# daac-tools/daachorse

Hardware: NVIDIA H100
Metric: input GB/s scanned, find_overlapping_iter, 675k-pat bytewise (higher is better)
Workload: dtype u8

## Files before the change

daachorse_b200/csrc/dev_image.cpp:

```cpp
#include "dev_image.h"

#include <algorithm>

namespace dach {

namespace {

bool fail_chains_terminate(const dach_pma* p, bool dead_is_terminal) {
    const size_t n = p->slots();
    std::vector<uint8_t> color(n, 0);
    std::vector<uint32_t> path;
    for (size_t start = 0; start < n; ++start) {
        if (color[start]) continue;
        path.clear();
        uint32_t s = uint32_t(start);
        for (;;) {
            if (s == kRoot || (dead_is_terminal && s == kDead) || color[s] == 2) break;
            if (color[s] == 1) return false;
            color[s] = 1;
            path.push_back(s);
            s = p->fail[s];
        }
        for (uint32_t v : path) color[v] = 2;
    }
// ... 155 lines not shown
        if (s != kRoot && s != kDead && !moved[s]) R->new_of_old[s] = uint32_t(s) + H;
        if (!rebased[s] && p->base[s] != 0) R->new_base[s] = p->base[s] + H;
    }
    R->vacant_check.assign(H, 0);
    for (uint32_t blk = 0; blk < H; blk += 256) {
        uint32_t ub = blk == 0 ? 0u : kNone;
        for (uint32_t b = blk; ub == kNone && b < blk + 256; ++b)
            if (!base_used[b]) {
                ub = b;
                break;
            }
        for (uint32_t v = blk; v < blk + 256; ++v)
            if (!used[v] || v == kRoot || v == kDead) R->vacant_check[v] = ub == kNone ? 0x100u : (0x100u | ((ub ^ v) & 0xffu));
    }
    R->hot_slots = H;
}

}

int build_image(const dach_pma* p, HostImage* img) {
    const size_t n = p->slots();
    const bool lm = is_leftmost(p->match_kind);
    img->charwise = p->charwise;
    img->match_kind = p->match_kind;
    img->n_slots = uint32_t(n);
    img->root_opos = n ? p->state_output_pos(kRoot) : 0;
    img->max_pattern_len = 0;
    for (const OutputRec& o : p->outputs)
        if (o.length > img->max_pattern_len) img->max_pattern_len = o.length;

// ... 76 lines not shown
                uint32_t check = p->opos_ch[s] & 0xffu;
                if (ns < H && R.vacant_check[ns]) check = R.vacant_check[ns] & 0xffu;
                r[0] = (R.new_base[s] << 8) | check;
                r[1] = (nid(f) << 8) | flags;
                const uint32_t list = opos ? img->outputs[(size_t)(opos - 1) * 4 + 3] : 0u;
                r[2] = (fbase << 8) | std::min<uint32_t>(list, 255u);
                r[3] = R.sig[s];
                img->opos_tab[ns] = opos;
            }
            for (uint32_t v = 0; v < H; ++v)
                if (R.vacant_check[v] && v != kRoot && v != kDead) img->crec[size_t(v) * 4] = R.vacant_check[v] & 0xffu;
            if (H)
                for (size_t s = 0; s < n; ++s)
                    if (R.new_of_old[s] < H) img->crec[(s + H) * 4] = p->opos_ch[s] & 0xffu;
        }
    } else {
        for (size_t s = 0; s < n; ++s) {
            uint32_t* r = &img->rec[s * 4];
            r[0] = p->base[s];
            r[1] = p->check[s];
            r[2] = p->fail[s];
            r[3] = p->output_pos[s];
        }
        img->root_table.assign(256, kRoot);
        img->mapper = p->mapper_table;
        img->root_base = n ? p->base[kRoot] : 0;
        if (n < (size_t(1) << 24) && p->outputs.size() < (size_t(1) << 24)) {
            auto skip_leaves = [&](uint32_t f) {
                while (f != kRoot && f != kDead && p->base[f] == 0) f = p->fail[f];
                return f;
// ... 34 lines not shown
```

daachorse_b200/csrc/dev_image.h:

```cpp
#pragma once

#include <cstdint>
#include <vector>

#include "host.h"

namespace dach {

struct HostImage {
    bool charwise = false;
    uint8_t match_kind = 0;
    uint32_t n_slots = 0;
    uint32_t root_opos = 0;
    uint32_t max_pattern_len = 0;
    std::vector<uint32_t> rec;
    std::vector<uint32_t> outputs;
    std::vector<uint32_t> root_table;
    std::vector<uint32_t> crec;
    std::vector<uint32_t> opos_tab;
    uint32_t root_base = 0;
    uint32_t want_hot_slots = 65536;
    uint32_t hot_slots = 0;
    uint32_t n_cslots = 0;
    std::vector<uint32_t> new_of_old;
    std::vector<uint32_t> old_of_new;
    std::vector<uint32_t> mapper;
    bool segmentable = false;
};

int build_image(const dach_pma* p, HostImage* img);

}
```

daachorse_b200/csrc/dev_scan.cu:

```cuda
#include <cuda_runtime.h>

#include <unistd.h>

#include <algorithm>
#include <atomic>
#include <chrono>
#include <cstdio>
#include <cstdlib>
#include <cstring>
#include <memory>
#include <mutex>
#include <string>
#include <vector>

#include "dev_image.h"
#include "host.h"
#include "scan_lane.cuh"

namespace dach {


constexpr int kMaxThreads = 1024;
constexpr int kMaxDevices = 64;
constexpr uint32_t kRootBytes = 1024;
// ... 167 lines not shown
                    }
                }
            }
        }
    }
    if constexpr (SINK::KIND == RK_HIST) {
        __syncthreads();
        for (uint32_t i = threadIdx.x; i < P.hist_smem; i += blockDim.x)
            if (E.s_cnt[i]) red_add_u64(P.slot_hist + i, E.s_cnt[i]);
    }
}

template <class M, class LANE, int MAXT, int MINB, bool HOT>
__global__ void __launch_bounds__(MAXT, MINB) k_scan_machine(ScanParams P) {
    if constexpr (M::QLEN)
        scan_machine<M, EventOps<M::ITER>, LANE, EventSink, HOT>(P);
    else
        scan_machine<M, M, LANE, Emitter, HOT>(P);
}
template <class M, class LANE, int MODE, int RK, bool HOT>
__global__ void __launch_bounds__(1024, 1) k_scan_machine_rk(ScanParams P) {
    scan_machine<M, SinkOps<M, MODE, RK>, LANE, SinkOf<RK>, HOT>(P);
}

template <int MODE, int MAXT, bool HOT>
__global__ void __launch_bounds__(MAXT, 1) k_scan_duo(ScanParams P) {
    using M = StdMachine3<MODE>;
    extern __shared__ __align__(128) unsigned char smem_raw[];
    uint4* s_hot = reinterpret_cast<uint4*>(smem_raw);
    QEntry* s_queue = reinterpret_cast<QEntry*>(smem_raw + (HOT ? (size_t)P.hot_entries * 16 : 0));
    __shared__ __align__(8) uint64_t s_bar;
// ... 598 lines not shown
    DevBuf counts, ev_counts, tiles, ctrl, pool;
    DevBuf nseg, seg_first, item_hay, item_beg, item_offs, n_items_dev;
    DevBuf blk_first, blkmap, tiles2;
    DevBuf stage;
    DevBuf items_rk, total_rk;
    DevBuf slot_hist, rec_hist, hist_acc;
    HostPinned* pinned = nullptr;
    cudaEvent_t ev[4] = {nullptr, nullptr, nullptr, nullptr};
    cudaEvent_t ev_scanned = nullptr, ev_placed = nullptr;
    cudaEvent_t ev_push[2] = {nullptr, nullptr};
    uint64_t job_n = 0, job_items = 0;
    uint32_t job_pool_blocks = 0;
    uint64_t job_cap = 0;
    bool job_seg = false, job_ordered = false, job_open = false, job_placed = false;
    bool job_events = false;
    bool refused = false;
    int job_mode = 0;
    cudaStream_t job_stream = nullptr;
    DevBuf text, offs, out, out_offs;
    void* offs_stage = nullptr;
    size_t offs_stage_bytes = 0;
    cudaStream_t stream = nullptr;
    bool init(bool with_stream) {
        if (!pinned && !cuda_ok(cudaMallocHost(reinterpret_cast<void**>(&pinned), sizeof(HostPinned)), "cudaMallocHost"))
            return false;
        for (int i = 0; i < 4; ++i)
            if (!ev[i] && !cuda_ok(cudaEventCreate(&ev[i]), "cudaEventCreate")) return false;
        if (!ev_scanned && !cuda_ok(cudaEventCreateWithFlags(&ev_scanned, cudaEventDisableTiming), "cudaEventCreate")) return false;
        if (!ev_placed && !cuda_ok(cudaEventCreateWithFlags(&ev_placed, cudaEventDisableTiming), "cudaEventCreate")) return false;
        for (int i = 0; i < 2; ++i)
// ... 44 lines not shown
    bool segmentable = false;
    uint32_t n_outputs = 0, max_value = 0, n_cslots = 0;
    size_t image_bytes = 0;
    int sm_count = 0;
    size_t smem_optin = 0;
    uint4* d_rec = nullptr;
    uint4* d_outputs = nullptr;
    uint32_t* d_root = nullptr;
    uint4* d_crec = nullptr;
    uint32_t* d_opos = nullptr;
    uint32_t* d_id_in = nullptr;
    uint32_t* d_id_out = nullptr;
    uint32_t hot_slots = 0;
    uint32_t root_base = 0;
    uint32_t* d_mapper = nullptr;
    void* image_base = nullptr;
    size_t image_alloc = 0;
    std::mutex mu;
    Workspace ws;
    static constexpr int kSlots = 4;
    Workspace slot[kSlots];
    int64_t opt_slice_mib = 64;
    int64_t opt_hot_entries = 6144;
    int64_t opt_hist_smem = 1024;
    int64_t opt_df_pairs = kDefaultDfPairs;
    int64_t opt_slice_ramp = 1;
    int64_t opt_tail_seg = 0;
    int64_t opt_gather_ordered = 1;
    int64_t opt_gather_u = 4;
    int64_t opt_reserve_sms = 0;
    int64_t opt_smem_pad_kib = 0;
    int64_t opt_seg_len = 0;
    int64_t opt_hot_records = 0;
    int64_t opt_threads = 1024;
    int64_t opt_ctas_per_sm = 1;
    int64_t opt_l2_hints = 2;
    int64_t opt_kernel = 3;
    std::atomic<uint64_t> launches{0};
    cudaEvent_t ev_ref = nullptr;
    double last_scan_ms = 0, last_total_ms = 0;
    uint64_t last_h2d = 0, last_d2h = 0;
    DevBuf df_tab[2], df_list[2], df_n, df_acc;
    uint32_t df_mask = 0, df_limit = 0;
    bool df_clean = false;
    uint64_t last_df_windows = 0, last_df_rescans = 0;
    std::atomic<int> refs{1};
};

struct dach_job {
    dach_dev* d = nullptr;
    Workspace W;
// ... 83 lines not shown
    return cudaGetLastError();
}
template <int MAXT, bool HOT>
cudaError_t launch_duo_m(int mode, const ScanParams& P, int grid, int threads, size_t smem, cudaStream_t st) {
    switch (mode) {
        case M_FIND: return launch_duo_t<M_FIND, MAXT, HOT>(P, grid, threads, smem, st);
        case M_NO_SUFFIX: return launch_duo_t<M_NO_SUFFIX, MAXT, HOT>(P, grid, threads, smem, st);
        case M_OVERLAPPING: return launch_duo_t<M_OVERLAPPING, MAXT, HOT>(P, grid, threads, smem, st);
    }
    return cudaErrorInvalidValue;
}
cudaError_t launch_duo(int mode, const ScanParams& P, int grid, int threads, size_t smem, cudaStream_t st) {
    if (threads > 768)
        return P.hot_entries ? launch_duo_m<1024, true>(mode, P, grid, threads, smem, st) : launch_duo_m<1024, false>(mode, P, grid, threads, smem, st);
    return P.hot_entries ? launch_duo_m<768, true>(mode, P, grid, threads, smem, st) : launch_duo_m<768, false>(mode, P, grid, threads, smem, st);
}

cudaError_t launch_cw(int mode, const ScanParams& P, int grid, int threads, size_t smem, cudaStream_t st) {
    switch (mode) {
        case M_FIND: return launch_machine_t<CwMachine<M_FIND>, LaneCw, 1024, 1, false>(P, grid, threads, smem, st);
        case M_OVERLAPPING: return launch_machine_t<CwMachine<M_OVERLAPPING>, LaneCw, 1024, 1, false>(P, grid, threads, smem, st);
        case M_NO_SUFFIX: return launch_machine_t<CwMachine<M_NO_SUFFIX>, LaneCw, 1024, 1, false>(P, grid, threads, smem, st);
        default: return launch_machine_t<CwMachine<M_LEFTMOST>, LaneCw, 1024, 1, false>(P, grid, threads, smem, st);
    }
}

cudaError_t launch_lm(const ScanParams& P, int grid, int threads, size_t smem, cudaStream_t st) {
    return launch_machine_t<LmMachine, LaneLm, 1024, 1, false>(P, grid, threads, smem, st);
}

// ... 121 lines not shown
    P.mapper = d->d_mapper;
    P.mapper_len = d->mapper_len;
    P.n_slots = d->n_slots;
    P.id_in = d->d_id_in;
    P.id_out = d->d_id_out;
    P.root_opos = d->root_opos;
    P.text = d_text;
    P.text_lo = text_lo;
    P.text_end = text_end;
    P.offs = d_offs;
    P.n_items = n;
    return P;
}

size_t plan_smem(const dach_dev* d, ScanParams& P, bool v1, bool std3, int threads, int ctas_per_sm, int queue_sets,
                 uint32_t hist_smem = 0) {
    const size_t smem_budget = std::min<size_t>(d->smem_optin, 226 * 1024) / ctas_per_sm - (ctas_per_sm > 1 ? 1024 : 0);
    size_t smem;
    if (v1) {
        const size_t queues = (size_t)LANE_Q * threads * sizeof(QEntry) * queue_sets + (size_t)hist_smem * 4;
        uint64_t want = 0;
        if (std3 && d->opt_hot_entries != 0 && smem_budget > queues + 512) {
            want = std::min<uint64_t>(d->hot_slots, (smem_budget - queues - 512) / 16);
            if (d->opt_hot_entries > 0) want = std::min<uint64_t>(want, (uint64_t)d->opt_hot_entries);
            want &= ~uint64_t(255);
        }
        smem = (size_t)want * 16 + queues;
        if (d->opt_smem_pad_kib > 0) smem = std::min<size_t>(smem + ((size_t)d->opt_smem_pad_kib << 10), smem_budget);
        P.hot_n = 0;
        P.hot_entries = (uint32_t)want;
    } else {
        uint64_t hot = smem_budget > kRootBytes ? (smem_budget - kRootBytes) / 16 : 0;
        if (d->opt_hot_records >= 0) hot = std::min<uint64_t>(hot, (uint64_t)d->opt_hot_records);
        hot = std::min<uint64_t>(hot, d->n_slots);
        P.hot_n = (uint32_t)hot;
        smem = kRootBytes + (size_t)hot * 16;
    }
    return smem;
// ... 48 lines not shown
        cudaEventRecord(W.ev_scanned, st);
        return DACH_OK;
    }
    int threads = (int)std::min<int64_t>(std::max<int64_t>(d->opt_threads, 32), kMaxThreads);
    threads = (threads / 32) * 32;
    int ctas_per_sm = (int)std::min<int64_t>(std::max<int64_t>(d->opt_ctas_per_sm, 1), 2048 / threads);
    const int free_sms = (int)std::min<int64_t>(std::max<int64_t>(d->opt_reserve_sms, 0), d->sm_count - 1);
    const int grid = (d->sm_count - free_sms) * ctas_per_sm;
    const bool v1 = d->opt_kernel >= 1 && d->d_crec && !(mode == M_FIND && d->root_opos != 0);
    const bool cw_machine = v1 && d->charwise;
    const bool lm_machine = v1 && !d->charwise && mode == M_LEFTMOST;
    const bool std2 = v1 && !d->charwise && mode != M_LEFTMOST && d->opt_kernel >= 2 && d->root_base != 0;
    const bool std3 = std2 && d->opt_kernel >= 3;
    const bool duo = std3 && d->opt_kernel >= 4 && ctas_per_sm == 1;
    const bool events = std3 && !duo;

    if (d_state_io && !std2 && !cw_machine) {
        set_error("stream chunks need a Standard lane machine (find / find_overlapping, at most 2^24 states, bytewise: "
                  "BASE(ROOT) != 0, no empty pattern for find)");
        return DACH_INVALID_ARGUMENT;
    }

    bool seg = v1 && !d->charwise && !d_state_io && (mode == M_OVERLAPPING || mode == M_NO_SUFFIX) && d->opt_seg_len >= 0 && d->segmentable;
    uint32_t seg_len = 0, seg_from = 0;
    uint64_t n_items_max = n;
    if (seg) {
        const uint64_t lanes = (uint64_t)grid * threads;
        const uint64_t warm = d->max_pattern_len ? d->max_pattern_len - 1 : 0;
        const uint64_t floor_len = std::max<uint64_t>(256, 8 * warm);
        uint64_t want;
// ... 26 lines not shown
    const uint32_t pool_blocks = (uint32_t)pool_blocks64;
    if (!ensure(W.counts, n_items_max * 4) || !ensure(W.tiles, n_tiles * 8) || !ensure(W.item_offs, (n_items_max + 1) * 8) ||
        !ensure(W.pool, (size_t)pool_blocks * BLK_WORDS * 4) || (events && !ensure(W.ev_counts, n_items_max * 4)))
        return DACH_CUDA_ERROR;
    if (seg && (!ensure(W.nseg, n * 4) || !ensure(W.seg_first, (n + 1) * 8) || !ensure(W.item_hay, n_items_max * 4) ||
                !ensure(W.item_beg, n_items_max * 4) || !ensure(W.n_items_dev, 8)))
        return DACH_CUDA_ERROR;

    ScanParams P = image_params(d, d_text, text_lo, text_end, d_offs, n);
    P.counts = static_cast<uint32_t*>(W.counts.p);
    P.ev_counts = events ? static_cast<uint32_t*>(W.ev_counts.p) : nullptr;
    P.pool = static_cast<uint32_t*>(W.pool.p);
    P.pool_blocks = pool_blocks;
    P.ctrl = static_cast<ScanCtrl*>(W.ctrl.p);
    P.state_io = d_state_io;
    const size_t smem = plan_smem(d, P, v1, std3, threads, ctas_per_sm, duo ? 2 : 1);

    unsigned long long* tiles = static_cast<unsigned long long*>(W.tiles.p);
    unsigned long long* item_offs = static_cast<unsigned long long*>(W.item_offs.p);
    k_check_offsets<<<(unsigned)((n + 255) / 256), 256, 0, st>>>(d_offs, n, (uint64_t)(text_end - d_text), P.ctrl);
    ++d->launches;
    if (seg) {
        cudaMemsetAsync(W.counts.p, 0, n_items_max * 4, st);
        if (events) cudaMemsetAsync(W.ev_counts.p, 0, n_items_max * 4, st);
        enqueue_seg_table(d, W, d_offs, n, seg_len, seg_from, P, st);
    }
    cudaEventRecord(W.ev[3], st);
    if (!cuda_ok(cw_machine   ? launch_cw(mode, P, grid, std::min(threads, 1024), smem, st)
                 : lm_machine ? launch_lm(P, grid, std::min(threads, 1024), smem, st)
                 : duo        ? launch_duo(mode, P, grid, threads, smem, st)
                 : v1         ? launch_std(std3 ? 3 : std2 ? 2 : 1, mode, P, grid, threads, smem, st,
                                           ctas_per_sm >= 2 && threads <= 768 && grid % 2 == 0)
                              : launch_scan(d->charwise, mode, P, grid, threads, smem, st),
                 "k_scan launch"))
        return DACH_CUDA_ERROR;
    cudaEventRecord(W.ev[1], st);
    k_offsets_tile_sums<1><<<(unsigned)n_tiles, kScanThreads, 0, st>>>(P.counts, n_items_max, tiles);
    k_offsets_scan_tiles<<<1, kScanThreads, 0, st>>>(tiles, n_tiles);
    k_offsets_apply<1><<<(unsigned)n_tiles, kScanThreads, 0, st>>>(P.counts, n_items_max, tiles, item_offs);
    d->launches += 4;
    const bool ordered = d->opt_gather_ordered >= 2 || (d->opt_gather_ordered == 1 && text_bytes >= (256ull << 20));
    if (ordered) {
        if (!ensure(W.blk_first, (n_items_max + 1) * 8) || !ensure(W.blkmap, (size_t)pool_blocks * 4) || !ensure(W.tiles2, n_tiles * 8))
// ... 6 lines not shown
            k_offsets_apply<BLK_EVENTS><<<(unsigned)n_tiles, kScanThreads, 0, st>>>(P.ev_counts, n_items_max, tiles2, blk_first);
        } else {
            k_offsets_tile_sums<BLK_MATCHES><<<(unsigned)n_tiles, kScanThreads, 0, st>>>(P.counts, n_items_max, tiles2);
            k_offsets_scan_tiles<<<1, kScanThreads, 0, st>>>(tiles2, n_tiles);
            k_offsets_apply<BLK_MATCHES><<<(unsigned)n_tiles, kScanThreads, 0, st>>>(P.counts, n_items_max, tiles2, blk_first);
        }
        k_blk_index<<<d->sm_count * 8, 256, 0, st>>>(P.pool, P.ctrl, pool_blocks, blk_first, static_cast<uint32_t*>(W.blkmap.p));
        d->launches += 4;
    }
    if (!cuda_ok(cudaGetLastError(), "kernel launch")) return DACH_CUDA_ERROR;
    cudaEventRecord(W.ev_scanned, st);
    W.job_items = n_items_max;
    W.job_seg = seg;
    W.job_ordered = ordered;
    W.job_events = events;
    W.job_mode = mode;
    W.job_pool_blocks = pool_blocks;
    return DACH_OK;
}

int enqueue_place(dach_dev* d, Workspace& W, dach_match* d_out, uint64_t out_cap, uint64_t* d_out_offs,
                  const unsigned long long* d_base, bool last, cudaStream_t st, const uint32_t* d_pos_in = nullptr,
                  bool staged = false, bool dma = false, uint64_t h_base = 0, uint64_t h_total = 0) {
    if (!W.job_open) {
        set_error("no scan to place");
        return DACH_INVALID_ARGUMENT;
    }
    if (st != W.job_stream) cudaStreamWaitEvent(st, W.ev_scanned, 0);
    const uint64_t n = W.job_n, n_items = W.job_items;
    const ScanCtrl* ctrl = static_cast<const ScanCtrl*>(W.ctrl.p);
// ... 4 lines not shown
        const uint32_t* pool = static_cast<const uint32_t*>(W.pool.p);
        const uint32_t* counts = static_cast<const uint32_t*>(W.counts.p);
        const uint32_t* blkmap = W.job_ordered ? static_cast<const uint32_t*>(W.blkmap.p) : nullptr;
        uint32_t* out_words = reinterpret_cast<uint32_t*>(d_out);
        const unsigned long long* g_base = d_base;
        unsigned long long g_cap = out_cap;
        if (staged) {
            if (!ensure(W.stage, W.job_cap * sizeof(dach_match) + 256)) return DACH_CUDA_ERROR;
            out_words = static_cast<uint32_t*>(W.stage.p);
            g_base = nullptr;
            g_cap = W.job_cap;
        }
        const unsigned long long* pad_like = staged ? d_base : nullptr;
        if (W.job_events) {
            const uint32_t* ev_counts = static_cast<const uint32_t*>(W.ev_counts.p);
            if (W.job_mode == M_OVERLAPPING)
                k_expand<true, 2><<<gather_grid, 256, 0, st>>>(pool, ctrl, W.job_pool_blocks, ev_counts, item_offs, n_items, g_cap, g_base,
                                                                out_words, blkmap, pad_like, d->d_outputs, d->d_opos);
            else
                k_expand<false, 2><<<gather_grid, 256, 0, st>>>(pool, ctrl, W.job_pool_blocks, ev_counts, item_offs, n_items, g_cap, g_base,
                                                                 out_words, blkmap, pad_like, d->d_outputs, d->d_opos);
        } else if (d->opt_gather_u >= 8)
            k_gather<8><<<gather_grid, 256, 0, st>>>(pool, ctrl, W.job_pool_blocks, counts, item_offs, n_items, g_cap, g_base, out_words, blkmap, pad_like);
        else if (d->opt_gather_u <= 2)
            k_gather<2><<<gather_grid, 256, 0, st>>>(pool, ctrl, W.job_pool_blocks, counts, item_offs, n_items, g_cap, g_base, out_words, blkmap, pad_like);
        else
            k_gather<4><<<gather_grid, 256, 0, st>>>(pool, ctrl, W.job_pool_blocks, counts, item_offs, n_items, g_cap, g_base, out_words, blkmap, pad_like);
        ++d->launches;
        if (staged) {
            cudaEventRecord(W.ev_push[0], st);
            if (dma) {
                if (h_total && h_base + h_total <= out_cap &&
                    !cuda_ok(cudaMemcpyAsync(reinterpret_cast<uint32_t*>(d_out) + h_base * 3ull, out_words + ((h_base * 3ull) & 3ull),
                                             h_total * sizeof(dach_match), cudaMemcpyDefault, st),
                             "peer copy"))
                    return DACH_CUDA_ERROR;
// ... 734 lines not shown
        d->device = device;
        d->charwise = img.charwise;
        d->match_kind = img.match_kind;
        d->n_slots = img.n_slots;
        d->root_opos = img.root_opos;
        d->max_pattern_len = img.max_pattern_len;
        d->segmentable = img.segmentable;
        d->mapper_len = (uint32_t)img.mapper.size();
        d->n_outputs = (uint32_t)(img.outputs.size() / 4);
        for (uint32_t i = 0; i < d->n_outputs; ++i) d->max_value = std::max(d->max_value, img.outputs[(size_t)i * 4]);
        d->n_cslots = (uint32_t)img.opos_tab.size();
        cudaDeviceProp prop;
        if (!cuda_ok(cudaGetDeviceProperties(&prop, device), "cudaGetDeviceProperties")) return DACH_CUDA_ERROR;
        d->sm_count = prop.multiProcessorCount;
        d->smem_optin = prop.sharedMemPerBlockOptin;
        constexpr int kParts = 8;
        const std::vector<uint32_t>* parts[kParts] = {&img.rec, &img.outputs, &img.root_table, &img.mapper, &img.crec, &img.opos_tab,
                                                       &img.new_of_old, &img.old_of_new};
        size_t part_off[kParts], total = 0;
        for (int i = 0; i < kParts; ++i) {
            part_off[i] = total;
            total += (std::max<size_t>(parts[i]->size() * 4, 16) + 511) & ~size_t(511);
            d->image_bytes += parts[i]->size() * 4;
        }
        bool ok = cuda_ok(cudaMalloc(&d->image_base, total), "cudaMalloc image");
        d->image_alloc = total;
        for (int i = 0; ok && i < kParts; ++i)
            if (!parts[i]->empty())
                ok = cuda_ok(cudaMemcpy(static_cast<char*>(d->image_base) + part_off[i], parts[i]->data(), parts[i]->size() * 4,
                                        cudaMemcpyHostToDevice),
                             "upload image");
        if (ok) {
            char* b = static_cast<char*>(d->image_base);
            d->d_rec = reinterpret_cast<uint4*>(b + part_off[0]);
            d->d_outputs = reinterpret_cast<uint4*>(b + part_off[1]);
            d->d_root = reinterpret_cast<uint32_t*>(b + part_off[2]);
            d->d_mapper = reinterpret_cast<uint32_t*>(b + part_off[3]);
            if (!img.crec.empty()) {
                d->d_crec = reinterpret_cast<uint4*>(b + part_off[4]);
                d->d_opos = reinterpret_cast<uint32_t*>(b + part_off[5]);
                if (img.hot_slots) {
                    d->d_id_in = reinterpret_cast<uint32_t*>(b + part_off[6]);
                    d->d_id_out = reinterpret_cast<uint32_t*>(b + part_off[7]);
                }
                d->hot_slots = img.hot_slots;
            }
            d->root_base = img.root_base;
        }
        ok = ok && install_policies((int)d->opt_l2_hints) && d->ws.init(false);
        if (!ok) {
            dach_dev_free(d.release());
            return DACH_CUDA_ERROR;
        }
        *out = d.release();
        return DACH_OK;
    });
}

void dach_dev_free(dach_dev* d) {
    if (!d || --d->refs > 0) return;
    DeviceGuard g(d->device);
    cudaFree(d->image_base);
// ... 523 lines not shown
        d->opt_tail_seg = value;
    else if (k == "gather_ordered")
        d->opt_gather_ordered = value;
    else if (k == "gather_u")
        d->opt_gather_u = value;
    else if (k == "reserve_sms")
        d->opt_reserve_sms = value;
    else if (k == "smem_pad_kib")
        d->opt_smem_pad_kib = value;
    else if (k == "hot_entries")
        d->opt_hot_entries = value;
    else if (k == "hist_smem")
        d->opt_hist_smem = value;
    else if (k == "df_pairs")
        d->opt_df_pairs = value;
    else if (k == "l2_hints") {
        d->opt_l2_hints = value;
        DeviceGuard g(d->device);
        if (!g.ok || !install_policies((int)value)) return DACH_CUDA_ERROR;
    } else {
        set_error("unknown option " + k);
        return DACH_INVALID_ARGUMENT;
    }
    return DACH_OK;
}

}
```

daachorse_b200/csrc/scan_lane.cuh:

```cuda
#pragma once

#include <stdint.h>

#include <type_traits>

#if defined(__CUDACC__)
#define DACH_HD __host__ __device__ __forceinline__
#else
#define DACH_HD inline
#ifndef DACH_EMU_TYPES
#define DACH_EMU_TYPES
struct uint4 {
    uint32_t x, y, z, w;
};
struct uint2 {
    uint32_t x, y;
};
#endif
#endif

#if defined(__CUDA_ARCH__)
#define DACH_SYNCWARP() __syncwarp()
#else
#define DACH_SYNCWARP()
// ... 1913 lines not shown
                L.sig = x.w;
                L.addr = st;
            }
            return;
        }
        if (MODE != M_FIND && (Ev.root_flags & CF_OUT) && beg == 0) {
            QEntry e;
            e.end = 0;
            e.opos = MODE == M_OVERLAPPING ? D_ROOT | (Ev.root_rec.z << 24) : D_ROOT;
            Ev.q[0] = e;
            L.qn = 1;
        }
    }
};

template <class M, int MODE, int RK>
struct SinkOps {
    using Sink = typename std::conditional<
        RK == RK_COUNT, CountSink,
        typename std::conditional<RK == RK_FIRST, FirstSink, typename std::conditional<RK == RK_HIST, HistSink, DfSink>::type>::type>::type;

    template <class LANE>
    static DACH_HD void begin_item(LANE& L, const ScanParams& P, const StdEnv& Ev, Sink& E, uint64_t item, const uint8_t* emu_lo) {
        Emitter unused;
        M::begin_item(L, P, Ev, unused, item, emu_lo);
        E.begin((uint32_t)item);
        if constexpr (RK == RK_DF) {
            if (P.item_hay) E.hay = P.item_hay[item];
        }
        if constexpr (RK == RK_FIRST) {
// ... 30 lines not shown
            L.qn = 0;
        } else {
            if (L.qn == (uint32_t)LANE_Q) {
                const QEntry e = Ev.q[(LANE_Q - 1) * Ev.q_stride];
                if (e.end >= L.from) {
                    emit_head(P, E, ld_u32(Ev.opos + (e.opos & QSLOT_MASK)), e.end);
                    L.fl |= F_DONE | M::IDLE;
                }
            }
            if (!(L.fl & F_DONE)) L.qn = (uint32_t)LANE_Q - 1;
        }
        if (!(L.fl & F_DONE)) L.fl &= ~M::IDLE;
    }
};

template <int MODE>
struct EventOps {
    using M = StdMachine3<MODE>;

    static DACH_HD void begin_item(Lane3& L, const ScanParams& P, const StdEnv& Ev, EventSink& E, uint64_t item,
                                   const uint8_t* emu_lo) {
        Emitter unused;
        M::begin_item(L, P, Ev, unused, item, emu_lo);
        E.begin((uint32_t)item);
    }

    static DACH_HD uint32_t reportable(const Lane3& L, const StdEnv& Ev) {
        uint32_t n = 0;
        for (uint32_t j = 0; j < (uint32_t)LANE_Q; ++j)
            if (j < L.qn && Ev.q[j * Ev.q_stride].end >= L.from) ++n;
        return n;
    }
    static DACH_HD bool need_block(const Lane3& L, const StdEnv& Ev, const EventSink& E) {
        return reportable(L, Ev) > BLK_EVENTS - E.fill;
    }

    static DACH_HD void drain(Lane3& L, const StdEnv& Ev, const ScanParams& P, EventSink& E, uint32_t blk) {
        for (uint32_t j = 0; j < (uint32_t)LANE_Q; ++j) {
            if (j < L.qn) {
                const QEntry e = Ev.q[j * Ev.q_stride];
                if (e.end >= L.from) {
                    if (E.fill == BLK_EVENTS) E.open(P, blk);
                    if (E.blk) st_stream_u2(E.blk + BLK_HDR_WORDS + 2 * E.fill, e.end, e.opos);
                    ++E.fill;
                    ++E.nev;
                    const uint32_t c = E.count + (MODE == M_OVERLAPPING ? qentry_len(P, Ev.opos, e.opos) : 1u);
                    if (c < E.count) count_carry(P);
                    E.count = c;
                }
            }
        }
        L.qn = 0;
// ... 6 lines not shown
```

Measured before the change: 122.9.

## Add UTF-8 codepoint-level automaton and lane machine for bytewise scans

Builds a second double-array automaton at the host whose transitions consume whole UTF-8 codepoints, remapped to frequency-ordered codes, when the bytewise trie is valid UTF-8 and the byte/boundary state ratio is high enough. A new Utf8Machine lane decodes one codepoint per step from a sliding 32-byte register window and walks this compressed trie, so fewer dependent state fetches are needed per input byte, and the smaller table fits the shared-memory hot cache better. It costs extra decode ALU work per step and a more complex host build, and it only applies to non-leftmost event-mode scans when the heuristic or option allows it.

```diff
diff --git a/daachorse_b200/csrc/dev_image.cpp b/daachorse_b200/csrc/dev_image.cpp
--- a/daachorse_b200/csrc/dev_image.cpp
+++ b/daachorse_b200/csrc/dev_image.cpp
@@ -193,6 +193,208 @@
             if (!used[v] || v == kRoot || v == kDead) R->vacant_check[v] = ub == kNone ? 0x100u : (0x100u | ((ub ^ v) & 0xffu));
     }
     R->hot_slots = H;
+}
+
+void build_utf8_image(const dach_pma* p, HostImage* img) {
+    const size_t n = p->slots();
+    img->u8_ok = false;
+    if (is_leftmost(p->match_kind) || n < 2 || img->root_opos != 0 || !img->segmentable) return;
+    auto child = [&](uint32_t s, uint32_t c) -> uint32_t {
+        const uint32_t b = p->base[s], ci = b ^ c;
+        return (b != 0 && ci < n && (p->opos_ch[ci] & 0xffu) == c) ? ci : kNone;
+    };
+    std::vector<uint8_t> rem(n, 0xff), lo(n, 0x80), hi(n, 0xbf);
+    std::vector<uint32_t> acc(n, 0), begin(n, kNone), bfs;
+    std::vector<uint32_t> cpar(n, kNone), cpt(n, 0);
+    bfs.push_back(kRoot);
+    rem[kRoot] = 0;
+    for (size_t h = 0; h < bfs.size(); ++h) {
+        const uint32_t s = bfs[h];
+        if (p->base[s] == 0) continue;
+        const uint32_t from = rem[s] == 0 ? s : begin[s];
+        for (uint32_t c = 0; c < 256; ++c) {
+            const uint32_t ci = child(s, c);
+            if (ci == kNone) continue;
+            uint32_t r;
+            if (rem[s] == 0) {
+                if (c < 0x80) {
+                    r = 0, acc[ci] = c;
+                } else if (c >= 0xc2 && c <= 0xdf) {
+                    r = 1, acc[ci] = c & 0x1f;
+                } else if (c >= 0xe0 && c <= 0xef) {
+                    r = 2, acc[ci] = c & 0x0f, lo[ci] = c == 0xe0 ? 0xa0 : 0x80, hi[ci] = c == 0xed ? 0x9f : 0xbf;
+                } else if (c >= 0xf0 && c <= 0xf4) {
+                    r = 3, acc[ci] = c & 0x07, lo[ci] = c == 0xf0 ? 0x90 : 0x80, hi[ci] = c == 0xf4 ? 0x8f : 0xbf;
+                } else {
+                    return;
+                }
+            } else {
+                if (c < lo[s] || c > hi[s]) return;
+                r = rem[s] - 1u;
+                acc[ci] = (acc[s] << 6) | (c & 0x3f);
+            }
+            rem[ci] = (uint8_t)r;
+            if (r == 0) {
+                cpar[ci] = from;
+                cpt[ci] = acc[ci];
+                begin[ci] = ci;
+            } else {
+                begin[ci] = from;
+            }
+            bfs.push_back(ci);
+        }
+    }
+    std::vector<uint32_t> bnd;
+    for (uint32_t s : bfs) {
+        if (rem[s] != 0) {
+            if (p->opos_ch[s] >> 8) return;
+            continue;
+        }
+        const uint32_t f = p->fail[s];
+        if (s != kRoot && (f >= n || rem[f] != 0)) return;
+        bnd.push_back(s);
+    }
+    if (bnd.size() < 2) return;
+    img->u8_ratio = double(bfs.size()) / double(bnd.size());
+
+    std::vector<std::pair<uint32_t, uint32_t>> freq;
+    {
+        std::vector<uint32_t> cps;
+        for (size_t i = 1; i < bnd.size(); ++i) cps.push_back(cpt[bnd[i]]);
+        std::sort(cps.begin(), cps.end());
+        for (size_t i = 0; i < cps.size();) {
+            size_t j = i;
+            while (j < cps.size() && cps[j] == cps[i]) ++j;
+            freq.push_back({uint32_t(j - i), cps[i]});
+            i = j;
+        }
+        std::stable_sort(freq.begin(), freq.end(), [](const std::pair<uint32_t, uint32_t>& a, const std::pair<uint32_t, uint32_t>& b) {
+            return a.first > b.first;
+        });
+    }
+    const uint32_t n_codes = uint32_t(freq.size());
+    if (n_codes >= 0xffffu) return;
+    uint32_t max_cp = 0;
+    for (auto& f : freq) max_cp = std::max(max_cp, f.second);
+    std::vector<uint32_t> mapper(size_t(max_cp) + 2, n_codes);
+    for (uint32_t k = 0; k < n_codes; ++k) mapper[freq[k].second] = k;
+
+    std::vector<uint32_t> code(n, 0), nch(n, 0), depth(n, 0), sub(n, 0);
+    for (size_t i = 1; i < bnd.size(); ++i) {
+        const uint32_t s = bnd[i];
+        code[s] = mapper[cpt[s]];
+        ++nch[cpar[s]];
+        depth[s] = depth[cpar[s]] + 1;
+    }
+    for (size_t i = bnd.size(); i-- > 0;) {
+        const uint32_t s = bnd[i];
+        sub[s] += 1;
+        if (s != kRoot) sub[cpar[s]] += sub[s];
+    }
+    std::vector<uint32_t> kid_off(n + 1, 0), kids(bnd.size() - 1);
+    for (size_t s = 0; s < n; ++s) kid_off[s + 1] = kid_off[s] + nch[s];
+    {
+        std::vector<uint32_t> fill(kid_off.begin(), kid_off.end() - 1);
+        for (size_t i = 1; i < bnd.size(); ++i) kids[fill[cpar[bnd[i]]]++] = bnd[i];
+    }
+    std::vector<uint32_t> par;
+    for (uint32_t s : bnd)
+        if (nch[s]) {
+            std::sort(kids.begin() + kid_off[s], kids.begin() + kid_off[s + 1], [&](uint32_t a, uint32_t b) { return code[a] < code[b]; });
+            par.push_back(s);
+        }
+    std::stable_sort(par.begin(), par.end(), [&](uint32_t a, uint32_t b) {
+        if (depth[a] != depth[b]) return depth[a] < depth[b];
+        return uint64_t(sub[a]) * nch[b] > uint64_t(sub[b]) * nch[a];
+    });
+
+    std::vector<uint32_t> nxt, nbase(n, 0), nid(n, kNone);
+    auto grow = [&](size_t want) {
+        size_t old = nxt.size();
+        if (want <= old) return;
+        want = std::max(want, old * 2);
+        nxt.resize(want);
+        for (size_t v = old; v < want; ++v) nxt[v] = uint32_t(v);
+    };
+    auto find = [&](uint32_t v) {
+        grow(size_t(v) + 2);
+        while (nxt[v] != v) {
+            nxt[v] = nxt[nxt[v]];
+            v = nxt[v];
+        }
+        return v;
+    };
+    auto is_free = [&](uint32_t v) { return find(v) == v; };
+    grow(size_t(n_codes) + 1024);
+    nxt[0] = 1;
+    nid[kRoot] = 0;
+    uint32_t top = 0, max_base = 0;
+    for (uint32_t s : par) {
+        const uint32_t* ks = &kids[kid_off[s]];
+        const uint32_t m = nch[s], kmin = code[ks[0]];
+        uint32_t b = kNone, v = find(kmin), tries = 0;
+        for (;;) {
+            const uint32_t cand = v - kmin;
+            bool ok = true;
+            for (uint32_t j = 1; ok && j < m; ++j) ok = is_free(cand + code[ks[j]]);
+            if (ok) {
+                b = cand;
+                break;
+            }
+            if (++tries > (1u << 20)) {
+                b = top + 1 - kmin;
+                break;
+            }
+            v = find(v + 1);
+        }
+        grow(size_t(b) + n_codes + 2);
+        nbase[s] = b;
+        max_base = std::max(max_base, b);
+        for (uint32_t j = 0; j < m; ++j) {
+            const uint32_t slot = b + code[ks[j]];
+            nxt[slot] = slot + 1;
+            nid[ks[j]] = slot;
+            top = std::max(top, slot);
+        }
+    }
+    const size_t N = std::max<size_t>(size_t(top) + 1, size_t(max_base) + n_codes + 1);
+    if (N >= kU24Max) return;
+
+    auto skip_leaves = [&](uint32_t f) {
+        while (f != kRoot && nch[f] == 0) f = p->fail[f];
+        return f;
+    };
+    img->u8_root_base = nbase[kRoot];
+    img->u8_codes = n_codes;
+    img->u8_crec.assign(N * 4, 0);
+    img->u8_opos.assign(N, 0);
+    img->u8_of_old.assign(n, kNone);
+    for (size_t v = 0; v < N; ++v) img->u8_crec[v * 4 + 3] = 0xffffffu << 8;
+    for (uint32_t s : bnd) {
+        const uint32_t ns = nid[s];
+        const uint32_t opos = p->opos_ch[s] >> 8;
+        const uint32_t f = skip_leaves(p->fail[s]);
+        uint32_t flags = opos ? 1u : 0u, fbase;
+        if (s == kRoot || f == kRoot) {
+            flags |= 8u;
+            fbase = img->u8_root_base;
+        } else {
+            fbase = nbase[f];
+            if (skip_leaves(p->fail[f]) == kRoot) flags |= 2u;
+        }
+        uint32_t sig = 0;
+        for (uint32_t j = kid_off[s]; j < kid_off[s + 1]; ++j) sig |= 1u << (code[kids[j]] & 15u);
+        const uint32_t list = opos ? img->outputs[(size_t)(opos - 1) * 4 + 3] : 0u;
+        uint32_t* r = &img->u8_crec[size_t(ns) * 4];
+        r[0] = (nbase[s] << 8) | (sig & 0xffu);
+        r[1] = (nid[f] << 8) | flags;
+        r[2] = (fbase << 8) | std::min<uint32_t>(list, 255u);
+        r[3] = ((s == kRoot ? 0xffffffu : nid[cpar[s]]) << 8) | (sig >> 8);
+        img->u8_opos[ns] = opos;
+        img->u8_of_old[s] = ns;
+    }
+    img->u8_mapper.swap(mapper);
+    img->u8_ok = true;
 }
 
 }
@@ -299,6 +501,7 @@
                 for (size_t s = 0; s < n; ++s)
                     if (R.new_of_old[s] < H) img->crec[(s + H) * 4] = p->opos_ch[s] & 0xffu;
         }
+        build_utf8_image(p, img);
     } else {
         for (size_t s = 0; s < n; ++s) {
             uint32_t* r = &img->rec[s * 4];
diff --git a/daachorse_b200/csrc/dev_image.h b/daachorse_b200/csrc/dev_image.h
--- a/daachorse_b200/csrc/dev_image.h
+++ b/daachorse_b200/csrc/dev_image.h
@@ -26,6 +26,14 @@
     std::vector<uint32_t> old_of_new;
     std::vector<uint32_t> mapper;
     bool segmentable = false;
+    bool u8_ok = false;
+    double u8_ratio = 0;
+    uint32_t u8_root_base = 0;
+    uint32_t u8_codes = 0;
+    std::vector<uint32_t> u8_crec;
+    std::vector<uint32_t> u8_opos;
+    std::vector<uint32_t> u8_mapper;
+    std::vector<uint32_t> u8_of_old;
 };
 
 int build_image(const dach_pma* p, HostImage* img);
diff --git a/daachorse_b200/csrc/dev_scan.cu b/daachorse_b200/csrc/dev_scan.cu
--- a/daachorse_b200/csrc/dev_scan.cu
+++ b/daachorse_b200/csrc/dev_scan.cu
@@ -205,7 +205,7 @@
 template <class M, class LANE, int MAXT, int MINB, bool HOT>
 __global__ void __launch_bounds__(MAXT, MINB) k_scan_machine(ScanParams P) {
     if constexpr (M::QLEN)
-        scan_machine<M, EventOps<M::ITER>, LANE, EventSink, HOT>(P);
+        scan_machine<M, EventOps<M::ITER, M, LANE>, LANE, EventSink, HOT>(P);
     else
         scan_machine<M, M, LANE, Emitter, HOT>(P);
 }
@@ -834,6 +834,7 @@
     uint64_t job_cap = 0;
     bool job_seg = false, job_ordered = false, job_open = false, job_placed = false;
     bool job_events = false;
+    bool job_u8 = false;
     bool refused = false;
     int job_mode = 0;
     cudaStream_t job_stream = nullptr;
@@ -908,6 +909,11 @@
     uint32_t hot_slots = 0;
     uint32_t root_base = 0;
     uint32_t* d_mapper = nullptr;
+    uint4* d_u8_crec = nullptr;
+    uint32_t* d_u8_opos = nullptr;
+    uint32_t* d_u8_mapper = nullptr;
+    uint32_t u8_slots = 0, u8_mapper_len = 0, u8_root_base = 0;
+    double u8_ratio = 0;
     void* image_base = nullptr;
     size_t image_alloc = 0;
     std::mutex mu;
@@ -929,6 +935,7 @@
     int64_t opt_threads = 1024;
     int64_t opt_ctas_per_sm = 1;
     int64_t opt_l2_hints = 2;
+    int64_t opt_utf8_stride = -1;
     int64_t opt_kernel = 3;
     std::atomic<uint64_t> launches{0};
     cudaEvent_t ev_ref = nullptr;
@@ -1042,6 +1049,21 @@
     if (threads > 768)
         return P.hot_entries ? launch_duo_m<1024, true>(mode, P, grid, threads, smem, st) : launch_duo_m<1024, false>(mode, P, grid, threads, smem, st);
     return P.hot_entries ? launch_duo_m<768, true>(mode, P, grid, threads, smem, st) : launch_duo_m<768, false>(mode, P, grid, threads, smem, st);
+}
+
+cudaError_t launch_utf8(int mode, const ScanParams& P, int grid, int threads, size_t smem, cudaStream_t st) {
+    switch (mode) {
+        case M_FIND:
+            return P.hot_entries ? launch_machine_t<Utf8Machine<M_FIND>, Lane8, 1024, 1, true>(P, grid, threads, smem, st)
+                                 : launch_machine_t<Utf8Machine<M_FIND>, Lane8, 1024, 1, false>(P, grid, threads, smem, st);
+        case M_NO_SUFFIX:
+            return P.hot_entries ? launch_machine_t<Utf8Machine<M_NO_SUFFIX>, Lane8, 1024, 1, true>(P, grid, threads, smem, st)
+                                 : launch_machine_t<Utf8Machine<M_NO_SUFFIX>, Lane8, 1024, 1, false>(P, grid, threads, smem, st);
+        case M_OVERLAPPING:
+            return P.hot_entries ? launch_machine_t<Utf8Machine<M_OVERLAPPING>, Lane8, 1024, 1, true>(P, grid, threads, smem, st)
+                                 : launch_machine_t<Utf8Machine<M_OVERLAPPING>, Lane8, 1024, 1, false>(P, grid, threads, smem, st);
+    }
+    return cudaErrorInvalidValue;
 }
 
 cudaError_t launch_cw(int mode, const ScanParams& P, int grid, int threads, size_t smem, cudaStream_t st) {
@@ -1193,14 +1215,14 @@
 }
 
 size_t plan_smem(const dach_dev* d, ScanParams& P, bool v1, bool std3, int threads, int ctas_per_sm, int queue_sets,
-                 uint32_t hist_smem = 0) {
+                 uint32_t hist_smem = 0, bool u8 = false) {
     const size_t smem_budget = std::min<size_t>(d->smem_optin, 226 * 1024) / ctas_per_sm - (ctas_per_sm > 1 ? 1024 : 0);
     size_t smem;
     if (v1) {
         const size_t queues = (size_t)LANE_Q * threads * sizeof(QEntry) * queue_sets + (size_t)hist_smem * 4;
         uint64_t want = 0;
         if (std3 && d->opt_hot_entries != 0 && smem_budget > queues + 512) {
-            want = std::min<uint64_t>(d->hot_slots, (smem_budget - queues - 512) / 16);
+            want = std::min<uint64_t>(u8 ? d->u8_slots : d->hot_slots, (smem_budget - queues - 512) / 16);
             if (d->opt_hot_entries > 0) want = std::min<uint64_t>(want, (uint64_t)d->opt_hot_entries);
             want &= ~uint64_t(255);
         }
@@ -1279,6 +1301,8 @@
     const bool std3 = std2 && d->opt_kernel >= 3;
     const bool duo = std3 && d->opt_kernel >= 4 && ctas_per_sm == 1;
     const bool events = std3 && !duo;
+    const bool u8 = events && !d_state_io && d->d_u8_crec &&
+                    (d->opt_utf8_stride > 0 || (d->opt_utf8_stride < 0 && d->u8_ratio >= 1.5));
 
     if (d_state_io && !std2 && !cw_machine) {
         set_error("stream chunks need a Standard lane machine (find / find_overlapping, at most 2^24 states, bytewise: "
@@ -1335,7 +1359,14 @@
     P.pool_blocks = pool_blocks;
     P.ctrl = static_cast<ScanCtrl*>(W.ctrl.p);
     P.state_io = d_state_io;
-    const size_t smem = plan_smem(d, P, v1, std3, threads, ctas_per_sm, duo ? 2 : 1);
+    if (u8) {
+        P.crec = d->d_u8_crec;
+        P.opos_tab = d->d_u8_opos;
+        P.root_base = d->u8_root_base;
+        P.mapper = d->d_u8_mapper;
+        P.mapper_len = d->u8_mapper_len;
+    }
+    const size_t smem = plan_smem(d, P, v1, std3, threads, ctas_per_sm, duo ? 2 : 1, 0, u8);
 
     unsigned long long* tiles = static_cast<unsigned long long*>(W.tiles.p);
     unsigned long long* item_offs = static_cast<unsigned long long*>(W.item_offs.p);
@@ -1347,7 +1378,8 @@
         enqueue_seg_table(d, W, d_offs, n, seg_len, seg_from, P, st);
     }
     cudaEventRecord(W.ev[3], st);
-    if (!cuda_ok(cw_machine   ? launch_cw(mode, P, grid, std::min(threads, 1024), smem, st)
+    if (!cuda_ok(u8           ? launch_utf8(mode, P, grid, threads, smem, st)
+                 : cw_machine ? launch_cw(mode, P, grid, std::min(threads, 1024), smem, st)
                  : lm_machine ? launch_lm(P, grid, std::min(threads, 1024), smem, st)
                  : duo        ? launch_duo(mode, P, grid, threads, smem, st)
                  : v1         ? launch_std(std3 ? 3 : std2 ? 2 : 1, mode, P, grid, threads, smem, st,
@@ -1384,6 +1416,7 @@
     W.job_seg = seg;
     W.job_ordered = ordered;
     W.job_events = events;
+    W.job_u8 = u8;
     W.job_mode = mode;
     W.job_pool_blocks = pool_blocks;
     return DACH_OK;
@@ -1418,12 +1451,13 @@
         const unsigned long long* pad_like = staged ? d_base : nullptr;
         if (W.job_events) {
             const uint32_t* ev_counts = static_cast<const uint32_t*>(W.ev_counts.p);
+            const uint32_t* opos = W.job_u8 ? d->d_u8_opos : d->d_opos;
             if (W.job_mode == M_OVERLAPPING)
                 k_expand<true, 2><<<gather_grid, 256, 0, st>>>(pool, ctrl, W.job_pool_blocks, ev_counts, item_offs, n_items, g_cap, g_base,
-                                                                out_words, blkmap, pad_like, d->d_outputs, d->d_opos);
+                                                                out_words, blkmap, pad_like, d->d_outputs, opos);
             else
                 k_expand<false, 2><<<gather_grid, 256, 0, st>>>(pool, ctrl, W.job_pool_blocks, ev_counts, item_offs, n_items, g_cap, g_base,
-                                                                 out_words, blkmap, pad_like, d->d_outputs, d->d_opos);
+                                                                 out_words, blkmap, pad_like, d->d_outputs, opos);
         } else if (d->opt_gather_u >= 8)
             k_gather<8><<<gather_grid, 256, 0, st>>>(pool, ctrl, W.job_pool_blocks, counts, item_offs, n_items, g_cap, g_base, out_words, blkmap, pad_like);
         else if (d->opt_gather_u <= 2)
@@ -2188,9 +2222,10 @@
         if (!cuda_ok(cudaGetDeviceProperties(&prop, device), "cudaGetDeviceProperties")) return DACH_CUDA_ERROR;
         d->sm_count = prop.multiProcessorCount;
         d->smem_optin = prop.sharedMemPerBlockOptin;
-        constexpr int kParts = 8;
-        const std::vector<uint32_t>* parts[kParts] = {&img.rec, &img.outputs, &img.root_table, &img.mapper, &img.crec, &img.opos_tab,
-                                                       &img.new_of_old, &img.old_of_new};
+        constexpr int kParts = 11;
+        const std::vector<uint32_t>* parts[kParts] = {&img.rec,        &img.outputs,    &img.root_table, &img.mapper,
+                                                       &img.crec,       &img.opos_tab,   &img.new_of_old, &img.old_of_new,
+                                                       &img.u8_crec,    &img.u8_opos,    &img.u8_mapper};
         size_t part_off[kParts], total = 0;
         for (int i = 0; i < kParts; ++i) {
             part_off[i] = total;
@@ -2220,6 +2255,15 @@
                 d->hot_slots = img.hot_slots;
             }
             d->root_base = img.root_base;
+            if (img.u8_ok) {
+                d->d_u8_crec = reinterpret_cast<uint4*>(b + part_off[8]);
+                d->d_u8_opos = reinterpret_cast<uint32_t*>(b + part_off[9]);
+                d->d_u8_mapper = reinterpret_cast<uint32_t*>(b + part_off[10]);
+                d->u8_slots = (uint32_t)img.u8_opos.size();
+                d->u8_mapper_len = (uint32_t)img.u8_mapper.size() - 1;
+                d->u8_root_base = img.u8_root_base;
+                d->u8_ratio = img.u8_ratio;
+            }
         }
         ok = ok && install_policies((int)d->opt_l2_hints) && d->ws.init(false);
         if (!ok) {
@@ -2773,6 +2817,8 @@
         d->opt_hist_smem = value;
     else if (k == "df_pairs")
         d->opt_df_pairs = value;
+    else if (k == "utf8_stride")
+        d->opt_utf8_stride = value;
     else if (k == "l2_hints") {
         d->opt_l2_hints = value;
         DeviceGuard g(d->device);
diff --git a/daachorse_b200/csrc/scan_lane.cuh b/daachorse_b200/csrc/scan_lane.cuh
--- a/daachorse_b200/csrc/scan_lane.cuh
+++ b/daachorse_b200/csrc/scan_lane.cuh
@@ -1951,6 +1951,190 @@
     }
 };
 
+
+struct Lane8 {
+    uint32_t hay_lo, hay_hi;
+    uint32_t ap, ap_end;
+    uint32_t t0, t1, t2, t3, t4, t5, t6, t7;
+    uint32_t r0, nf, r2;
+    uint32_t sig;
+    uint32_t cu;
+    uint32_t addr;
+    uint32_t qn, fl, item;
+    uint32_t from;
+};
+
+DACH_HD uint32_t utf8_unit(uint32_t t0, uint32_t t1, uint32_t t2, uint32_t t3, uint32_t t4, uint32_t t5, uint32_t o,
+                           const uint32_t* mapper, uint32_t mapper_len) {
+    const uint32_t w = o >> 2;
+    const uint32_t a = w == 0 ? t0 : w == 1 ? t1 : w == 2 ? t2 : w == 3 ? t3 : t4;
+    const uint32_t b = w == 0 ? t1 : w == 1 ? t2 : w == 2 ? t3 : w == 3 ? t4 : t5;
+    const uint32_t x = (uint32_t)((((uint64_t)b << 32) | a) >> ((o & 3u) * 8u));
+    const uint32_t b0 = x & 0xffu;
+    const uint32_t need = b0 < 0xc0u ? 0u : b0 < 0xe0u ? 1u : b0 < 0xf0u ? 2u : b0 < 0xf8u ? 3u : 0u;
+    const uint32_t cm = (((x & 0xc0c0c000u) ^ 0x80808000u) >> 8) | 0x01000000u;
+#if defined(__CUDA_ARCH__)
+    const uint32_t run_all = (uint32_t)(__ffs((int)cm) - 1) >> 3;
+#else
+    const uint32_t run_all = (uint32_t)__builtin_ctz(cm) >> 3;
+#endif
+    const uint32_t run = run_all < need ? run_all : need;
+    const uint32_t c1 = (x >> 8) & 0x3fu, c2 = (x >> 16) & 0x3fu, c3 = (x >> 24) & 0x3fu;
+    const uint32_t cp = need == 0 ? b0
+                        : need == 1 ? ((b0 & 0x1fu) << 6) | c1
+                        : need == 2 ? ((b0 & 0x0fu) << 12) | (c1 << 6) | c2
+                                    : ((b0 & 0x07u) << 18) | (c1 << 12) | (c2 << 6) | c3;
+    const uint32_t cp_min = need == 0 ? 0u : need == 1 ? 0x80u : need == 2 ? 0x800u : 0x10000u;
+    const bool ok = run == need && (b0 < 0x80u || b0 >= 0xc0u) && b0 < 0xf8u && cp >= cp_min && cp < mapper_len;
+    const uint32_t code = ld_u32(mapper + (ok ? cp : mapper_len));
+    return code | ((run + 1u) << 16);
+}
+
+template <int MODE>
+struct Utf8Machine {
+    static constexpr int TOPUP = 8;
+    static constexpr bool LAZY = true;
+    static constexpr bool LEAN = true;
+    static constexpr uint32_t IDLE = F3_STOP;
+    static constexpr bool QLEN = true;
+    static constexpr int ITER = MODE;
+
+    static DACH_HD uint4 fetch(const StdEnv& Ev, uint32_t a) { return StdMachine3<MODE>::fetch(Ev, a); }
+    static DACH_HD const uint8_t* window_of(const Lane8& L) {
+        const uint64_t hi = (uint64_t)(L.hay_hi + (L.ap < L.hay_lo ? 1u : 0u));
+        return reinterpret_cast<const uint8_t*>((uintptr_t)((hi << 32) | (L.ap & ~15u)));
+    }
+    static DACH_HD void load_next(Lane8& L, const StdEnv& Ev, const uint8_t* q) {
+#if defined(__CUDA_ARCH__)
+        const uint32_t inside = q >= Ev.text_lo && q + 16 <= Ev.text_end;
+        asm volatile("{\n\t.reg .pred p;\n\tsetp.ne.u32 p, %4, 0;\n\t"
+                     "@p ld.global.nc.L2::cache_hint.v4.u32 {%0,%1,%2,%3}, [%5], %6;\n\t}"
+                     : "+r"(L.t4), "+r"(L.t5), "+r"(L.t6), "+r"(L.t7)
+                     : "r"(inside), "l"(q), "l"(c_l2pol[1]));
+        if (inside) return;
+#endif
+        uint2 w = ld_text8_safe(q, Ev.text_lo, Ev.text_end);
+        L.t4 = w.x, L.t5 = w.y;
+        w = ld_text8_safe(q + 8, Ev.text_lo, Ev.text_end);
+        L.t6 = w.x, L.t7 = w.y;
+    }
+    static DACH_HD void text_topup(Lane8&, const StdEnv&, const uint8_t*) {}
+    static DACH_HD void adopt(Lane8& L, const uint4& x) {
+        L.r0 = x.x;
+        L.nf = x.y;
+        L.r2 = x.z;
+        L.sig = (x.x & 0xffu) | ((x.w & 0xffu) << 8);
+    }
+    static DACH_HD void to_root(Lane8& L, const StdEnv& Ev) {
+        adopt(L, Ev.root_rec);
+        L.addr = D_ROOT;
+    }
+    static DACH_HD uint32_t next_unit(const Lane8& L, const StdEnv& Ev) {
+        return utf8_unit(L.t0, L.t1, L.t2, L.t3, L.t4, L.t5, (L.ap & 15u) + (L.cu >> 16), Ev.mapper, Ev.mapper_len);
+    }
+
+    static DACH_HD void land(Lane8& L, const StdEnv& Ev, uint32_t nu) {
+        const uint32_t o = (L.ap & 15u) + (L.cu >> 16);
+        L.ap += L.cu >> 16;
+        L.cu = nu;
+        if (o >= 16u) {
+            L.t0 = L.t4, L.t1 = L.t5, L.t2 = L.t6, L.t3 = L.t7;
+            load_next(L, Ev, window_of(L) + 16);
+        }
+        if (L.ap_end - L.ap < (nu >> 16)) L.fl |= F_DONE | F3_STOP;
+        if (L.nf & CF_OUT) {
+            DACH_STAT(pushes);
+            QEntry e;
+            e.end = L.ap - L.hay_lo;
+            e.opos = MODE == M_OVERLAPPING ? L.addr | (L.r2 << 24) : L.addr;
+            Ev.q[L.qn * Ev.q_stride] = e;
+            if (++L.qn == (uint32_t)LANE_Q) L.fl |= F3_STOP;
+            if (MODE == M_FIND) to_root(L, Ev);
+        }
+    }
+
+    static DACH_HD bool step(Lane8& L, const StdEnv& Ev, const uint8_t* emu_lo = nullptr) {
+        (void)emu_lo;
+        if (L.fl & F3_STOP) return false;
+        const uint32_t k = L.cu & 0xffffu;
+        const uint32_t bit = 1u << (k & 15u);
+        const uint32_t own = L.sig & bit;
+        const uint32_t a = (((own ? L.r0 : L.r2) >> 8) + k) & QSLOT_MASK;
+        const uint4 x = fetch(Ev, a);
+        const uint32_t nu = next_unit(L, Ev);
+        DACH_STAT(steps);
+        if (L.fl & F3_LEARN) {
+            DACH_STAT(learns);
+            L.nf = x.y;
+            L.r2 = x.z;
+            L.sig &= ~bit;
+            L.fl &= ~F3_LEARN;
+            return true;
+        }
+        DACH_STAT(probes);
+        if ((x.w >> 8) == (own ? L.addr : L.nf >> 8)) {
+            DACH_STAT(hits);
+            adopt(L, x);
+            L.addr = a;
+            land(L, Ev, nu);
+        } else if (own) {
+            DACH_STAT(miss_known);
+            L.sig &= ~bit;
+        } else if (L.nf & CF_FROOT) {
+            DACH_STAT(root_stay);
+            to_root(L, Ev);
+            land(L, Ev, nu);
+        } else if (L.nf & CF_F2ROOT) {
+            DACH_STAT(miss_f2root);
+            L.r2 = Ev.root_base << 8;
+            L.nf = (L.nf & 0xffu) | CF_FROOT;
+        } else {
+            L.r0 = ((L.nf >> 8) - k) << 8;
+            L.sig |= bit;
+            L.fl |= F3_LEARN;
+        }
+        return true;
+    }
+
+    static DACH_HD void finish_item(const Lane8&, const ScanParams&) {}
+
+    static DACH_HD void begin_item(Lane8& L, const ScanParams& P, const StdEnv& Ev, Emitter& E, uint64_t item,
+                                   const uint8_t* emu_lo) {
+        (void)emu_lo;
+        uint64_t hay = item;
+        uint32_t beg = 0;
+        if (P.item_hay) {
+            hay = P.item_hay[item];
+            beg = P.item_beg[item];
+        }
+        const uint64_t o0 = P.offs[hay], o1 = P.offs[hay + 1];
+        const uint32_t hay_len = (uint32_t)(o1 - o0);
+        const uintptr_t h = (uintptr_t)(P.text + o0);
+        L.hay_lo = (uint32_t)h;
+        L.hay_hi = (uint32_t)((uint64_t)h >> 32);
+        uint32_t start = 0, end = hay_len;
+        if (P.item_hay && hay >= P.seg_from) {
+            const uint64_t e64 = (uint64_t)beg + P.seg_len;
+            if (e64 < hay_len) end = (uint32_t)e64;
+            start = beg > P.warm ? beg - P.warm : 0;
+        }
+        L.ap = L.hay_lo + start;
+        L.ap_end = L.hay_lo + end;
+        L.from = beg ? beg + 1 : 0;
+        L.item = (uint32_t)item;
+        L.qn = 0;
+        E.begin((uint32_t)item);
+        const uint8_t* w0 = window_of(L);
+        load_next(L, Ev, w0);
+        L.t0 = L.t4, L.t1 = L.t5, L.t2 = L.t6, L.t3 = L.t7;
+        load_next(L, Ev, w0 + 16);
+        L.cu = 0;
+        L.cu = next_unit(L, Ev);
+        to_root(L, Ev);
+        L.fl = F_ACTIVE | (start >= end || L.ap_end - L.ap < (L.cu >> 16) ? (F_DONE | F3_STOP) : 0u);
+    }
+};
+
 template <class M, int MODE, int RK>
 struct SinkOps {
     using Sink = typename std::conditional<
@@ -2011,28 +2195,26 @@
     }
 };
 
-template <int MODE>
+template <int MODE, class M = StdMachine3<MODE>, class LANE = Lane3>
 struct EventOps {
-    using M = StdMachine3<MODE>;
-
-    static DACH_HD void begin_item(Lane3& L, const ScanParams& P, const StdEnv& Ev, EventSink& E, uint64_t item,
+    static DACH_HD void begin_item(LANE& L, const ScanParams& P, const StdEnv& Ev, EventSink& E, uint64_t item,
                                    const uint8_t* emu_lo) {
         Emitter unused;
         M::begin_item(L, P, Ev, unused, item, emu_lo);
         E.begin((uint32_t)item);
     }
 
-    static DACH_HD uint32_t reportable(const Lane3& L, const StdEnv& Ev) {
+    static DACH_HD uint32_t reportable(const LANE& L, const StdEnv& Ev) {
         uint32_t n = 0;
         for (uint32_t j = 0; j < (uint32_t)LANE_Q; ++j)
             if (j < L.qn && Ev.q[j * Ev.q_stride].end >= L.from) ++n;
         return n;
     }
-    static DACH_HD bool need_block(const Lane3& L, const StdEnv& Ev, const EventSink& E) {
+    static DACH_HD bool need_block(const LANE& L, const StdEnv& Ev, const EventSink& E) {
         return reportable(L, Ev) > BLK_EVENTS - E.fill;
     }
 
-    static DACH_HD void drain(Lane3& L, const StdEnv& Ev, const ScanParams& P, EventSink& E, uint32_t blk) {
+    static DACH_HD void drain(LANE& L, const StdEnv& Ev, const ScanParams& P, EventSink& E, uint32_t blk) {
         for (uint32_t j = 0; j < (uint32_t)LANE_Q; ++j) {
             if (j < L.qn) {
                 const QEntry e = Ev.q[j * Ev.q_stride];
```

Result: faster. 128.3, median of 6 (+4.4%).
